# antofuller/jumbo_mae_tpu

Hardware: AMD Instinct MI355X
Metric: pretrain images/sec (whole node) ViT-L/16 224 mask75% at 1/2/4/8 MI355X (higher is better)
Workload: dtype bf16; 1 GPU; model=vit_large_patch16 jumbo-MAE (3 CLS, shared jumbo MLP) + decoder 8x512x16h, global_batch=4096, seq_len=52, decoder_seq_len=199, parallelism=dp1, per_gpu_batch=4096, grad_accum=2, micro_batch=2048, grad_ckpt=False, hip_graph=False, optimizer=adamw(0.9,0.95) wd0.05 warmup-cosine

## Files before the change

jumbo_mae_tpu_amd/csrc/bindings.cpp:

```cpp
#include <torch/extension.h>
#include <c10/hip/HIPStream.h>
#include <hip/hip_runtime.h>

#include <climits>

#include "jm_api.h"

namespace {

hipStream_t stream() { return c10::hip::getCurrentHIPStream().stream(); }

#define CHECK_CUDA(x) TORCH_CHECK((x).is_cuda(), #x " must be a GPU tensor")
#define CHECK_CONTIG(x) TORCH_CHECK((x).is_contiguous(), #x " must be contiguous")
#define CHECK_DT(x, d) TORCH_CHECK((x).scalar_type() == (d), #x " has wrong dtype")

const uint16_t* bf(const torch::Tensor& t) { return reinterpret_cast<const uint16_t*>(t.data_ptr()); }
uint16_t* bfm(torch::Tensor& t) { return reinterpret_cast<uint16_t*>(t.data_ptr()); }
uint16_t* bfp(const torch::Tensor& t) { return reinterpret_cast<uint16_t*>(t.data_ptr()); }
const float* fopt(const c10::optional<torch::Tensor>& t) {
  return t.has_value() && t->defined() ? t->data_ptr<float>() : nullptr;
}
float* fopt_m(c10::optional<torch::Tensor>& t) { return t.has_value() && t->defined() ? t->data_ptr<float>() : nullptr; }

void check_rc(int rc, const char* what) { TORCH_CHECK(rc == 0, what, ": unsupported shape (rc=", rc, ")"); }
// ... 1546 lines not shown
  m.def("attn_max_seq", &jm_attn_max_seq);
  m.def("attn_head_dims", &attn_head_dims);
  m.def("attn_fused_bias", &attn_fused_bias, py::arg("S"), py::arg("hd"));
  m.def("attn_dropout", &attn_dropout, py::arg("S"), py::arg("hd"));
  m.def("gemm_tn_wgrad", &gemm_tn_wgrad, py::arg("dy"), py::arg("x"), py::arg("g"), py::arg("store") = false);
  m.def("gemm_tn_wgrad_seg", &gemm_tn_wgrad_seg, py::arg("dys"), py::arg("xs"), py::arg("g"), py::arg("store") = false);
  m.def("zero_ranges", &zero_ranges, "zero float ranges of a flat buffer (one launch)");
  m.def("colsum_add_f32", &colsum_add_f32, "g += x.sum(0) for a row-strided fp32 [rows, n] view");
  m.def("gemm_tn_wgrad_seg_group", &gemm_tn_wgrad_seg_group, py::arg("dys"), py::arg("xs"), py::arg("gs"),
        py::arg("stores") = std::vector<bool>{}, "grouped segmented weight gradients (<= 2 problems)");
  m.def("gemm_tn_wgrad_group", &gemm_tn_wgrad_group, py::arg("dys"), py::arg("xs"), py::arg("gs"),
        py::arg("stores") = std::vector<bool>{}, "grouped weight gradients over one M (<= 4 problems)");
  m.def("gemm_test_force", &jm_gemm_test_force, py::arg("path"), py::arg("rows") = 0,
        "numerics tests only: NT GEMM kernel path 0 = by shape, 1 = 64-deep main loop everywhere, "
        "2 = 4-phase kernels at every M without tail split (rows = forced tile height)");
  m.def("gemm_nt_tiles", &jm_gemm_nt_tiles, py::arg("M"), py::arg("N"), py::arg("K") = 1024, py::arg("epi") = 0,
        py::arg("lda") = 0, "output tiles (workgroups before split-K) of an NT launch");
  m.def(
      "gemm_nt_tail_plan",
      [](int M, int N, int K, int epi, long lda) {
        int r = 0;
        long n = 0;
        const int S = jm_gemm_nt_tail_plan(M, N, K, epi, lda, &r, &n);
        return std::make_pair(S, r);
      },
      py::arg("M"), py::arg("N"), py::arg("K"), py::arg("epi") = 0, py::arg("lda") = 0,
      "(S, tail tiles) of the tail split of an NT launch (S = 0: none); read-only");
  m.def("transpose_bf16_batch", &transpose_bf16_batch);
  m.def("gemm_nt_splitk", &gemm_nt_splitk, py::arg("A"), py::arg("B"), py::arg("bias") = py::none(),
        py::arg("splits") = 8, py::arg("add") = py::none());
// ... 62 lines not shown
```

jumbo_mae_tpu_amd/csrc/common.h:

```cpp
#pragma once
#include <hip/hip_runtime.h>
#include <hip/hip_bf16.h>
#include <stdint.h>

#include "jm_api.h"

#define JM_DEVICE __device__ __forceinline__

typedef __attribute__((ext_vector_type(8))) __bf16 bf16x8_t;
typedef __attribute__((ext_vector_type(4))) float f32x4_t;
typedef __attribute__((ext_vector_type(4))) short s16x4_t;
typedef __attribute__((ext_vector_type(8))) short s16x8_t;
typedef uint16_t bf16_raw;

constexpr int WAVE = 64;

JM_DEVICE float bf2f(uint16_t v) { return __uint_as_float(((uint32_t)v) << 16); }

JM_DEVICE uint32_t drop_hash(uint32_t j, uint64_t seed) {
  uint32_t x = (j + (uint32_t)seed) ^ (uint32_t)(seed >> 32);
  x ^= x >> 16;
  x *= 0x7feb352du;
  x ^= x >> 15;
  x *= 0x846ca68bu;
// ... 95 lines not shown
template <int B>
JM_DEVICE uint32_t gd_put(float d, uint32_t w) { return __builtin_amdgcn_cvt_pk_u8_f32(__builtin_fmaf(d, GD_Q, (float)GD_Z), B, w); }
JM_DEVICE uint2 gd_pack8(const float* d) {
  uint2 v;
  v.x = gd_put<3>(d[3], gd_put<2>(d[2], gd_put<1>(d[1], gd_put<0>(d[0], 0u))));
  v.y = gd_put<3>(d[7], gd_put<2>(d[6], gd_put<1>(d[5], gd_put<0>(d[4], 0u))));
  return v;
}
JM_DEVICE void gd_unpack4(uint32_t w, float s, float* d) {
  d[0] = ((float)(w & 255u) - (float)GD_Z) * s;
  d[1] = ((float)((w >> 8) & 255u) - (float)GD_Z) * s;
  d[2] = ((float)((w >> 16) & 255u) - (float)GD_Z) * s;
  d[3] = ((float)(w >> 24) - (float)GD_Z) * s;
}

template <int CTRL>
JM_DEVICE float dpp_mov(float v) {
  return __builtin_bit_cast(float, __builtin_amdgcn_update_dpp(0, __builtin_bit_cast(int, v), CTRL, 0xF, 0xF, true));
}

template <int CTRL>
JM_DEVICE uint32_t dpp_mov_u32(uint32_t v) {
  return (uint32_t)__builtin_amdgcn_update_dpp(0, (int)v, CTRL, 0xF, 0xF, true);
}

JM_DEVICE float row16_sum(float v) {
  v += dpp_mov<0xB1>(v);
  v += dpp_mov<0x4E>(v);
  v += dpp_mov<0x141>(v);
  v += dpp_mov<0x140>(v);
// ... 111 lines not shown
```

jumbo_mae_tpu_amd/csrc/gemm.hip:

```cpp
#include <type_traits>

#include "common.h"
#include "jm_api.h"

namespace {

constexpr int BM = 256, BN = 256;
constexpr size_t GEMM_SMEM = 128 * 1024;

typedef __attribute__((address_space(3))) void lds_void_t;

JM_DEVICE __amdgpu_buffer_rsrc_t make_rsrc(const uint16_t* base, long bytes) {
  const int n = bytes >= 0xffffffffL ? -1 : (int)bytes;
  return __builtin_amdgcn_make_buffer_rsrc((void*)base, (short)0, n, 0x00020000);
}

JM_DEVICE void blds16(__amdgpu_buffer_rsrc_t r, uint32_t voff, uint32_t soff, uint16_t* l) {
  __builtin_amdgcn_raw_ptr_buffer_load_lds(r, (lds_void_t*)(l), 16, voff, soff, 0, 0);
}

JM_DEVICE bf16x8_t lds8(const uint16_t* p) { return *reinterpret_cast<const bf16x8_t*>(p); }

JM_DEVICE f32x4_t mfma16(bf16x8_t a, bf16x8_t b, f32x4_t c) {
  return __builtin_amdgcn_mfma_f32_16x16x32_bf16(a, b, c, 0, 0, 0);
// ... 12 lines not shown

namespace {

template <int W>
JM_DEVICE void gelu_d_drop(const GemmEpi& ep, long idx0, float* g, float* d) {
  const uint64_t seed = (uint64_t)ep.dseed[0];
#pragma unroll
  for (int j = 0; j < W; j += 2) {
    const uint32_t h = drop_hash((uint32_t)((idx0 + j) >> 1), seed);
    const bool k0 = drop_keep_half(h, 0, ep.dthr), k1 = drop_keep_half(h, 1, ep.dthr);
    g[j] = k0 ? g[j] * ep.dscale : 0.f;
    d[j] = k0 ? d[j] : 0.f;
    g[j + 1] = k1 ? g[j + 1] * ep.dscale : 0.f;
    d[j + 1] = k1 ? d[j + 1] : 0.f;
  }
}

template <int EPI, int NTW, int MTW = 8>
JM_DEVICE void epilogue(const f32x4_t (&acc)[8][NTW], const GemmEpi& ep, int M, int N, int mb, int nb, int l16,
                        int g) {
#pragma unroll
  for (int nt = 0; nt < NTW; ++nt) {
    const int n = nb + nt * 16 + 4 * g;
    if (n >= N) continue;
    float bv[4] = {0.f, 0.f, 0.f, 0.f};
    if (ep.bias) load4(ep.bias + n, bv);
#pragma unroll
    for (int mt = 0; mt < MTW; ++mt) {
      const int m = mb + mt * 16 + l16;
      if (m >= M) continue;
// ... 64 lines not shown
}

template <typename T>
JM_DEVICE void st16(T* p, uint4 v, bool nts) {
  typedef __attribute__((ext_vector_type(4))) unsigned int u32x4_t;
  if (nts) __builtin_nontemporal_store(u32x4_t{v.x, v.y, v.z, v.w}, reinterpret_cast<u32x4_t*>(p));
  else *reinterpret_cast<uint4*>(p) = v;
}

JM_DEVICE void st8(uint8_t* p, uint2 v, bool nts) {
  typedef __attribute__((ext_vector_type(2))) unsigned int u32x2_t;
  if (nts) __builtin_nontemporal_store(u32x2_t{v.x, v.y}, reinterpret_cast<u32x2_t*>(p));
  else *reinterpret_cast<uint2*>(p) = v;
}

JM_DEVICE uint4 pack8(const float* f) {
  uint4 v;
  v.x = pack_bf2(f[0], f[1]);
  v.y = pack_bf2(f[2], f[3]);
  v.z = pack_bf2(f[4], f[5]);
  v.w = pack_bf2(f[6], f[7]);
  return v;
}

template <int EPI, int NTW, int NTH, int BNT = BN, bool NTS = false, int TR = BM>
JM_DEVICE void epilogue_lds(const f32x4_t (&acc)[8][NTW], const GemmEpi& ep, uint16_t* cs, int M, int N, int m0,
                            int n0, int wr, int wc, int l16, int g) {
  constexpr int RB = BNT;
  constexpr int HR = TR / 2, MTW = HR / 16;
  asm volatile("s_waitcnt vmcnt(0) lgkmcnt(0)\n\ts_barrier" ::: "memory");
  constexpr int LPR = BNT / 8;
  constexpr int RPP = NTH / LPR;
  int tid = threadIdx.x;
  asm volatile("" : "+v"(tid));
  const int c = tid % LPR;
  const bool col_ok = n0 + c * 8 < N;
  constexpr bool PRE = EPI == EPI_DGELU || EPI == EPI_DMUL;
  constexpr int NPASS = PRE ? TR / RPP : 1;
  constexpr int PF = NPASS < 8 ? NPASS : 8;
  uint4 auxv[PF];
  auto aux_load = [&](int i) {
    const int m = m0 + tid / LPR + i * RPP;
// ... 48 lines not shown
        }
        uint4 o;
        uint32_t* ow = reinterpret_cast<uint32_t*>(&o);
#pragma unroll
        for (int j = 0; j < 8; j += 2) {
          const float a0 = bf2f(dg[j]) * (EPI == EPI_DMUL ? hp[j] : gd[j]);
          const float a1 = bf2f(dg[j + 1]) * (EPI == EPI_DMUL ? hp[j + 1] : gd[j + 1]);
          ow[j / 2] = pack_bf2(a0, a1);
          f[j] = __uint_as_float(ow[j / 2] << 16);
          f[j + 1] = __uint_as_float(ow[j / 2] & 0xffff0000u);
          csum[j] += f[j];
          csum[j + 1] += f[j + 1];
        }
        st16(ep.out + (long)m * ep.ldo + n0 + c * 8, o, NTS);
      } else if (EPI == EPI_GELU_D) {
        float fh[8], fg[8], fd[8];
        const uint16_t* h = reinterpret_cast<const uint16_t*>(&v);
#pragma unroll
        for (int j = 0; j < 8; ++j) fh[j] = bf2f(h[j]);
        gelu_n<8, true, true>(fh, fg, fd);
        if (ep.dseed) gelu_d_drop<8>(ep, (long)m * ep.ldo + n0 + c * 8, fg, fd);
        st8(ep.dq + (long)m * ep.ldo + n0 + c * 8, gd_pack8(fd), NTS);
        st16(ep.out2 + (long)m * ep.ldo + n0 + c * 8, pack8(fg), NTS);
      } else if (EPI == EPI_GELU_ONLY) {
        float fh[8], f[8];
        const uint16_t* h = reinterpret_cast<const uint16_t*>(&v);
#pragma unroll
        for (int j = 0; j < 8; ++j) fh[j] = bf2f(h[j]);
        gelu_n<8, true, false>(fh, f, nullptr);
        st16(ep.out + (long)m * ep.ldo + n0 + c * 8, pack8(f), NTS);
      } else {
        st16(ep.out + (long)m * ep.ldo + n0 + c * 8, v, NTS);
      }
      if (EPI == EPI_GELU) {
        float fh[8], f[8];
        const uint16_t* h = reinterpret_cast<const uint16_t*>(&v);
#pragma unroll
        for (int j = 0; j < 8; ++j) fh[j] = bf2f(h[j]);
        gelu_n<8, true, false>(fh, f, nullptr);
        st16(ep.out2 + (long)m * ep.ldo + n0 + c * 8, pack8(f), NTS);
      }
    }
  };
  if constexpr (PRE) {
#pragma unroll
    for (int i = 0; i < NPASS; ++i) {
      pass(tid / LPR + i * RPP, auxv[i % PF]);
      if (i + PF < NPASS) auxv[i % PF] = aux_load(i + PF);
    }
  } else {
#pragma unroll 4
    for (int r = tid / LPR; r < TR; r += RPP) pass(r, auxv[0]);
  }
  if ((EPI == EPI_DGELU || EPI == EPI_DMUL) && ep.colpart != nullptr) {
    float* red = reinterpret_cast<float*>(cs);
    __syncthreads();
// ... 107 lines not shown
      __builtin_amdgcn_sched_barrier(0);
      if constexpr (KIND == 2) issue(u + 2);
      read(u + 1, H0{}, f0);
      mfma_rows(R4{}, f1);
      interleave();
    } else {
      mfma_rows(R4{}, f1);
    }
    __builtin_amdgcn_sched_barrier(0);
  };
  using K2 = std::integral_constant<int, 2>;
  using K1 = std::integral_constant<int, 1>;
  using K0 = std::integral_constant<int, 0>;

  const int nst = K / BK2;
  issue(0);
  if (nst > 1) {
    issue(1);
    asm volatile("s_waitcnt vmcnt(8)\n\ts_barrier" ::: "memory");
  } else {
    asm volatile("s_waitcnt vmcnt(0)\n\ts_barrier" ::: "memory");
  }
  __builtin_amdgcn_sched_barrier(0);
  Frags<NTW> f0, f1;
  read(0, H0{}, f0);
  int u = 0;
  for (; u + 2 < nst; ++u) stage(K2{}, u, f0, f1);
  if (u + 1 < nst) stage(K1{}, u++, f0, f1);
  stage(K0{}, u, f0, f1);

// ... 12 lines not shown
  } else if (EPI == EPI_PARTIAL) {
    float* dst = ep.part + (long)split * M * N;
#pragma unroll
    for (int mt = 0; mt < 8; ++mt) {
      const int m = m0 + wr * 128 + mt * 16 + l16;
      if (m >= M) continue;
#pragma unroll
      for (int nt = 0; nt < NTW; ++nt) {
        const int n = n0 + wc * NTW * 16 + nt * 16 + 4 * g;
        if (n >= N) continue;
        float v[4] = {acc[mt][nt][0], acc[mt][nt][1], acc[mt][nt][2], acc[mt][nt][3]};
        store4(dst + (long)m * N + n, v);
      }
    }
  } else if (N % 8 == 0)
    epilogue_lds<EPI, NTW, 512, BN, NTS>(acc, ep, smem, M, N, m0, n0, wr, wc, l16, g);
  else
    epilogue<EPI, NTW>(acc, ep, M, N, m0 + wr * 128, n0 + wc * NTW * 16, l16, g);
}

template <int EPI, bool NTS>
__global__ __launch_bounds__(512, 1) void gemm_nt64_kernel(const uint16_t* __restrict__ A, long lda,
                                                           const uint16_t* __restrict__ B, long ldb, int M, int N,
                                                           int K, GemmEpi ep, int GROUP_M) {
  JM_DGUARD(blockDim.x == 512 && K % 64 == 0 && M > 0 && N > 0);
  extern __shared__ __attribute__((aligned(16))) uint16_t smem[];
  nt64_body<EPI, NTS>(A, lda, B, ldb, M, N, K, ep, GROUP_M, smem);
}

template <int MTL>
__attribute__((always_inline)) JM_DEVICE void p4_mainloop(const uint16_t* __restrict__ A, long lda,
// ... 147 lines not shown
  sync(I3{});
  issue(1, I2{});
  read_a(0, I0{}, ax);
  read_b(0, I0{}, bp);
  int t = 0;
  for (; t + 4 <= nk; t += 2) {
    tile(K2{}, t, bp, bq);
    tile(K2{}, t + 1, bq, bp);
  }
  tile(K1{}, t, bp, bq);
  tile(K0{}, t + 1, bq, bp);
}

template <int EPI, int MTL>
__attribute__((always_inline)) JM_DEVICE void p4_epilogue(const f32x4_t (&acc)[8][4], const GemmEpi& ep, int M,
                                                          int N, int m0, int n0, int split, uint16_t* smem) {
  constexpr int NTW = 4, WN = 4;
  constexpr int HR = 64 + 16 * MTL, MTW = 4 + MTL;
  const int tid = threadIdx.x;
  const int wave = __builtin_amdgcn_readfirstlane(tid >> 6), lane = tid & 63;
  const int l16 = lane & 15, g = lane >> 4;
  const int wr = wave / WN, wc = wave % WN;
  if (EPI == EPI_PARTIAL) {
    float* dst = ep.part + (long)split * M * N;
#pragma unroll
    for (int mt = 0; mt < MTW; ++mt) {
      const int m = m0 + wr * HR + mt * 16 + l16;
      if (m >= M) continue;
#pragma unroll
      for (int nt = 0; nt < NTW; ++nt) {
        const int n = n0 + wc * NTW * 16 + nt * 16 + 4 * g;
        if (n >= N) continue;
        float v[4] = {acc[mt][nt][0], acc[mt][nt][1], acc[mt][nt][2], acc[mt][nt][3]};
        store4(dst + (long)m * N + n, v);
      }
    }
  } else if (N % 8 == 0)
    epilogue_lds<EPI, NTW, 512, BN, true, 2 * HR>(acc, ep, smem, M, N, m0, n0, wr, wc, l16, g);
  else
    epilogue<EPI, NTW, MTW>(acc, ep, M, N, m0 + wr * HR, n0 + wc * NTW * 16, l16, g);
}

template <int EPI, int MTL = 4>
__global__ __launch_bounds__(512, 1) void gemm_p4_kernel(const uint16_t* __restrict__ A, long lda,
                                                         const uint16_t* __restrict__ B, long ldb, int M, int N,
                                                         int K, GemmEpi ep, int GROUP_M) {
  JM_DGUARD(blockDim.x == 512 && K % 128 == 0 && M > 0 && N > 0);
  extern __shared__ __attribute__((aligned(16))) uint16_t smem[];
  if (__builtin_amdgcn_readfirstlane(threadIdx.x) >= 256) __builtin_amdgcn_s_setprio(1);
  int m0, n0, split = 0;
  if (EPI != EPI_PARTIAL && ep.t_count > 0) {
    int tg;
    tile_of_range(M, N, GROUP_M, ep.t_begin, ep.t_count, 1, m0, n0, split, tg);
  } else {
    tile_of<BN, 128 + 32 * MTL>(M, N, GROUP_M, m0, n0, EPI == EPI_PARTIAL ? ep.splits : 1,
                                EPI == EPI_PARTIAL ? &split : nullptr);
  }
  int k_begin = 0;
  if (EPI == EPI_PARTIAL) {
    const int ku = K / 128;
    const int ku0 = split * ku / ep.splits, ku1 = (split + 1) * ku / ep.splits;
    k_begin = ku0 * 128;
    K = (ku1 - ku0) * 128;
  }
  f32x4_t acc[8][4];
  p4_mainloop<MTL>(A, lda, B, ldb, M, N, m0, n0, k_begin, K, acc, smem);
  p4_epilogue<EPI, MTL>(acc, ep, M, N, m0, n0, split, smem);
}

constexpr int NBM = 128, NBN = 192, NKT = 64;
constexpr int N_AEL = NBM * NKT, N_BEL = NBN * NKT, N_STAGE = N_AEL + N_BEL;
constexpr int N_RING = 3;
constexpr int N_LD = NBN + 8;
static_assert(N_RING * N_STAGE * 2 <= (int)GEMM_SMEM, "narrow ring exceeds the LDS budget");

JM_DEVICE void narrow_tile(int M, int N, int GROUP_M, int splits, int& m0, int& n0, int& split) {
  const int nM = (M + NBM - 1) / NBM, nN = (N + NBN - 1) / NBN;
  const int tiles = nM * nN, nwg = tiles * splits;
  const int orig = blockIdx.x;
  const int xcd = orig & 7, q = nwg >> 3, r = nwg & 7;
  int wg = (xcd < r ? xcd * (q + 1) : r * (q + 1) + (xcd - r) * q) + (orig >> 3);
  split = wg / tiles;
  wg -= split * tiles;
  const int per_group = GROUP_M * nN;
  const int first_m = (wg / per_group) * GROUP_M;
  const int gsz = min(nM - first_m, GROUP_M);
  m0 = (first_m + (wg % per_group) % gsz) * NBM;
  n0 = ((wg % per_group) / gsz) * NBN;
}

template <int EPI>
JM_DEVICE void narrow_epilogue(const f32x4_t (&acc)[4][3], const GemmEpi& ep, uint16_t* cs, int M, int N, int m0,
                               int n0, int split, int wr, int wc, int l16, int g) {
  if constexpr (EPI == EPI_PARTIAL) {
    float* dst = ep.part + (long)split * M * N;
#pragma unroll
    for (int mt = 0; mt < 4; ++mt) {
      const int m = m0 + wr * 64 + mt * 16 + l16;
      if (m >= M) continue;
#pragma unroll
      for (int nt = 0; nt < 3; ++nt) {
        const int n = n0 + wc * 48 + nt * 16 + 4 * g;
        if (n >= N) continue;
        float v[4] = {acc[mt][nt][0], acc[mt][nt][1], acc[mt][nt][2], acc[mt][nt][3]};
        store4(dst + (long)m * N + n, v);
      }
    }
    return;
// ... 52 lines not shown
          gd_unpack4(auxv[i].x, ep.dqs, hp);
          gd_unpack4(auxv[i].y, ep.dqs, hp + 4);
        } else {
          const uint16_t* ah = reinterpret_cast<const uint16_t*>(&auxv[i]);
#pragma unroll
          for (int j = 0; j < 8; ++j) hp[j] = bf2f(ah[j]);
          gelu_n<8, false, true>(hp, nullptr, gd);
        }
#pragma unroll
        for (int j = 0; j < 8; ++j) {
          f[j] = bf2f(f2bf(bf2f(h[j]) * (EPI == EPI_DMUL ? hp[j] : gd[j])));
          csum[j] += f[j];
        }
        st16(o, pack8(f), false);
      } else if constexpr (EPI == EPI_GELU_D) {
        float fh[8], fg[8], fd[8];
#pragma unroll
        for (int j = 0; j < 8; ++j) fh[j] = bf2f(h[j]);
        gelu_n<8, true, true>(fh, fg, fd);
        if (ep.dseed) gelu_d_drop<8>(ep, (long)m * ep.ldo + n, fg, fd);
        st8(ep.dq + (long)m * ep.ldo + n, gd_pack8(fd), false);
        st16(ep.out2 + (long)m * ep.ldo + n, pack8(fg), false);
      } else if constexpr (EPI == EPI_GELU_ONLY) {
        float fh[8], f[8];
#pragma unroll
        for (int j = 0; j < 8; ++j) fh[j] = bf2f(h[j]);
        gelu_n<8, true, false>(fh, f, nullptr);
        st16(o, pack8(f), false);
      } else {
        st16(o, v, false);
        if constexpr (EPI == EPI_GELU) {
          float fh[8], f[8];
#pragma unroll
          for (int j = 0; j < 8; ++j) fh[j] = bf2f(h[j]);
          gelu_n<8, true, false>(fh, f, nullptr);
          st16(ep.out2 + (long)m * ep.ldo + n, pack8(f), false);
        }
      }
    }
  }
  if constexpr (PRE) {
    if (ep.colpart != nullptr) {
      float* red = reinterpret_cast<float*>(cs);
      __syncthreads();
      if (active) {
#pragma unroll
        for (int j = 0; j < 8; ++j) red[rr * NBN + c * 8 + j] = csum[j];
      }
      __syncthreads();
      if (tid < NBN && n0 + tid < N) {
        float a = 0.f;
#pragma unroll
// ... 43 lines not shown
    uint16_t* lb = la + N_AEL;
#pragma unroll
    for (int p = 0; p < 2; ++p) blds16(ra, a_src[p], k0b, la + (wave + 8 * p) * 8 * NKT);
#pragma unroll
    for (int p = 0; p < 3; ++p) blds16(rb, b_src[p], k0b, lb + (wave + 8 * p) * 8 * NKT);
  };
  const int ch0 = ((0 * 4 + g) ^ swz64(l16)) * 8, ch1 = ((1 * 4 + g) ^ swz64(l16)) * 8;
  const int a_row = (wr * 64 + l16) * NKT, b_row = N_AEL + (wc * 48 + l16) * NKT;
  f32x4_t acc[4][3];
#pragma unroll
  for (int i = 0; i < 4; ++i)
#pragma unroll
    for (int j = 0; j < 3; ++j) acc[i][j] = f32x4_t{0.f, 0.f, 0.f, 0.f};

  const int nk = K / NKT;
  issue(0);
  if (nk > 1) issue(1);
  for (int t = 0; t < nk; ++t) {
    if (t + 1 < nk) asm volatile("s_waitcnt vmcnt(5) lgkmcnt(0)\n\ts_barrier" ::: "memory");
    else asm volatile("s_waitcnt vmcnt(0) lgkmcnt(0)\n\ts_barrier" ::: "memory");
    __builtin_amdgcn_sched_barrier(0);
    if (t + 2 < nk) issue(t + 2);
    const uint16_t* base = smem + (t % N_RING) * N_STAGE;
    bf16x8_t a[4][2], b[3][2];
#pragma unroll
    for (int kk = 0; kk < 2; ++kk) {
      const int ch = kk ? ch1 : ch0;
#pragma unroll
      for (int nt = 0; nt < 3; ++nt) b[nt][kk] = lds8(base + b_row + nt * 16 * NKT + ch);
#pragma unroll
// ... 3 lines not shown
    for (int kk = 0; kk < 2; ++kk)
#pragma unroll
      for (int mt = 0; mt < 4; ++mt)
#pragma unroll
        for (int nt = 0; nt < 3; ++nt) acc[mt][nt] = mfma16(b[nt][kk], a[mt][kk], acc[mt][nt]);
    __builtin_amdgcn_sched_group_barrier(0x100, 7, 0);
#pragma unroll
    for (int i = 0; i < 7; ++i) {
      __builtin_amdgcn_sched_group_barrier(0x008, 1, 0);
      __builtin_amdgcn_sched_group_barrier(0x100, 1, 0);
    }
    __builtin_amdgcn_sched_group_barrier(0x008, 17, 0);
    __builtin_amdgcn_sched_barrier(0);
  }
  if (wave >= 4) __builtin_amdgcn_s_setprio(0);
  narrow_epilogue<EPI>(acc, ep, smem, M, N, m0, n0, split, wr, wc, l16, g);
}

template <int EPI>
__global__ __launch_bounds__(256) void tail_finish_kernel(GemmEpi ep, int M, int N, int GROUP_M) {
  __shared__ float red[8][BN];
  const int tg = blockIdx.x >> 3, rb = blockIdx.x & 7;
  int m0, n0;
  tile_coords(ep.t_begin + tg, M, N, GROUP_M, m0, n0);
  const int tid = threadIdx.x, c = tid & 31, rr = tid >> 5;
  const int n = n0 + c * 8;
  float csum[8] = {0.f, 0.f, 0.f, 0.f, 0.f, 0.f, 0.f, 0.f};
  float bv[8] = {0.f, 0.f, 0.f, 0.f, 0.f, 0.f, 0.f, 0.f};
  if (ep.bias && n < N) load8(ep.bias + n, bv);
#pragma unroll
  for (int i = 0; i < 4; ++i) {
// ... 61 lines not shown
    int dev = 0;
    (void)hipGetDevice(&dev);
    hipDeviceProp_t prop;
    (void)hipGetDeviceProperties(&prop, dev);
    g_num_cus = prop.multiProcessorCount;
  }
  return g_num_cus;
}

template <int EPI, bool NTS>
void launch_nt64(const uint16_t* A, long lda, const uint16_t* B, long ldb, int M, int N, int K, const GemmEpi& ep,
                 int nwg, hipStream_t st) {
  static bool attr = false;
  if (!attr) {
    (void)hipFuncSetAttribute((const void*)gemm_nt64_kernel<EPI, NTS>, hipFuncAttributeMaxDynamicSharedMemorySize,
                              (int)GEMM_SMEM);
    attr = true;
  }
  gemm_nt64_kernel<EPI, NTS><<<nwg, 512, GEMM_SMEM, st>>>(A, lda, B, ldb, M, N, K, ep, GEMM_GROUP);
}

template <int EPI, int MTL>
void launch_p4(const uint16_t* A, long lda, const uint16_t* B, long ldb, int M, int N, int K, const GemmEpi& ep,
               int nwg, hipStream_t st) {
  static bool attr = false;
  if (!attr) {
    (void)hipFuncSetAttribute((const void*)gemm_p4_kernel<EPI, MTL>, hipFuncAttributeMaxDynamicSharedMemorySize,
                              (int)GEMM_SMEM);
    attr = true;
  }
  gemm_p4_kernel<EPI, MTL><<<nwg, 512, GEMM_SMEM, st>>>(A, lda, B, ldb, M, N, K, ep, GEMM_GROUP);
}

template <int EPI>
void launch_narrow(const uint16_t* A, long lda, const uint16_t* B, long ldb, int M, int N, int K, const GemmEpi& ep,
                   hipStream_t st) {
  static bool attr = false;
  constexpr size_t sm = (size_t)N_RING * N_STAGE * 2;
  if (!attr) {
    (void)hipFuncSetAttribute((const void*)gemm_narrow_kernel<EPI>, hipFuncAttributeMaxDynamicSharedMemorySize,
                              (int)sm);
    attr = true;
  }
  const int nwg = ((M + NBM - 1) / NBM) * ((N + NBN - 1) / NBN) * (EPI == EPI_PARTIAL ? ep.splits : 1);
  gemm_narrow_kernel<EPI><<<nwg, 512, sm, st>>>(A, lda, B, ldb, M, N, K, ep, GEMM_GROUP);
}

constexpr int NARROW_MAX_M = 4096;

bool p4_ok(int K, int epi, int splits) {
  return g_test_path != 1 && K % 128 == 0 && (epi != EPI_PARTIAL || K / 128 >= splits);
}

// ... 55 lines not shown

template <int EPI>
void launch_tail(const uint16_t* A, long lda, const uint16_t* B, long ldb, int M, int N, int K, const GemmEpi& ep,
                 int tiles, hipStream_t st) {
  const int r = ep.t_count;
  GemmEpi em = ep;
  em.t_begin = 0;
  em.t_count = tiles - r;
  launch_epi<EPI>(A, lda, B, ldb, M, N, K, em, tiles - r, st);
  GemmEpi et = ep;
  et.t_begin = tiles - r;
  launch_nt64<EPI_TAIL, false>(A, lda, B, ldb, M, N, K, et, r * ep.tail_S, st);
  tail_finish_kernel<EPI><<<r * 8, 256, 0, st>>>(et, M, N, GEMM_GROUP);
}

}

void jm_gemm_test_force(int path, int rows) {
  g_test_path = (path == 1 || path == 2) ? path : 0;
  g_test_rows = (g_test_path == 2 && (rows == 224 || rows == 192 || rows == 160 || rows == 256)) ? rows : 0;
}

int jm_gemm_nt_tiles(int M, int N, int K, int epi, long lda) {
  if (narrow(M, N, K, epi)) return ((M + NBM - 1) / NBM) * ((N + NBN - 1) / NBN);
  const int tr = tile_rows(M, N, K, epi, lda);
  return ((M + tr - 1) / tr) * ((N + BN - 1) / BN);
}

int jm_gemm_nt_colpart_rows(int M, int N, int K, int epi, long lda) {
  if (narrow(M, N, K, epi)) return (M + NBM - 1) / NBM;
// ... 19 lines not shown
  *tail_r = r;
  return S;
}
}

int jm_gemm_nt_tail_plan(int M, int N, int K, int epi, long lda, int* tail_r, long* ws_floats) {
  *tail_r = 0;
  *ws_floats = 0;
  if (tile_rows(M, N, K, epi, lda) != BM) return 0;
  const int S = tail_plan_256(M, N, K, epi, tail_r);
  *ws_floats = (long)S * *tail_r * BM * BN;
  return S;
}

int jm_gemm_nt(const uint16_t* A, long lda, const uint16_t* B, long ldb, int M, int N, int K, int epi,
               const GemmEpi& ep, hipStream_t st) {
  if (K % 64 || N % 4 || M <= 0 || N <= 0) return -1;
  if ((long)M * lda * 2 >= (1L << 32) || (long)N * ldb * 2 >= (1L << 32)) return -2;
  const int nwg = ((M + BM - 1) / BM) * ((N + BN - 1) / BN) * (epi == EPI_PARTIAL ? ep.splits : 1);
  if (epi == EPI_PARTIAL && (ep.splits < 1 || (K / 64) < ep.splits)) return -4;
  if (ep.tail != nullptr && ep.tail_S >= 2 && ep.t_count > 0) {
    const int tiles = ((M + BM - 1) / BM) * ((N + BN - 1) / BN);
    if (epi == EPI_STORE) launch_tail<EPI_STORE>(A, lda, B, ldb, M, N, K, ep, tiles, st);
    else if (epi == EPI_GELU) launch_tail<EPI_GELU>(A, lda, B, ldb, M, N, K, ep, tiles, st);
    else if (epi == EPI_DGELU) launch_tail<EPI_DGELU>(A, lda, B, ldb, M, N, K, ep, tiles, st);
    else if (epi == EPI_GELU_ONLY) launch_tail<EPI_GELU_ONLY>(A, lda, B, ldb, M, N, K, ep, tiles, st);
    else return -3;
    return 0;
  }
  if (epi == EPI_PARTIAL)
    launch_epi<EPI_PARTIAL>(A, lda, B, ldb, M, N, K, ep, nwg, st);
  else if (epi == EPI_STORE)
// ... 18 lines not shown
```

jumbo_mae_tpu_amd/csrc/jm_api.h:

```cpp
#pragma once
#include <cstddef>
#include <cstdint>

#include <hip/hip_runtime.h>

struct JmDrop {
  const int64_t* seed;
  uint32_t thr;
  float scale;
  long ioff;
};

struct JmLnRes {
  const uint16_t* y;
  uint16_t* dy;
  long yB, yT;
  const float* scale;
  const float* mask;
  int T0;
  float* dscale;
  float* dbias;
  JmDrop drop;
};

// ... 21 lines not shown
  uint16_t* out2;
  const uint16_t* aux;
  float* colpart;
  float* part;
  int splits;
  float* tail;
  int tail_S;
  int t_begin;
  int t_count;
  const int64_t* dseed;
  uint32_t dthr;
  float dscale;
  uint8_t* dq;
  const uint8_t* dqa;
  float dqs;
};


int jm_layernorm_fwd(const float* x, long sB, long sT, int B, int T, int D, const float* gamma, const float* beta,
                     float eps, void* y, int out_bf16, float* mean, float* rstd, hipStream_t st, uint16_t* y2 = nullptr);
int jm_layernorm_bwd(const void* dy, int dy_bf16, const float* x, long sB, long sT, int B, int T, int D,
                     const float* mean, const float* rstd, const float* gamma, float* dx_ptr, long oB, long oT,
                     const float* dres, long rB, long rT, float* dgamma, float* dbeta, int accum_params, float* ws,
                     const JmLnRes* res, hipStream_t st, const uint16_t* hx = nullptr,
                     const float* beta = nullptr);
int jm_layernorm_bwd_blocks(int rows, int D);
int jm_residual_ln_fwd(const float* x, long sB, long sT, const uint16_t* y, const float* scale, const float* mask,
                       float* x1, long oB, long oT, uint16_t* h, float* mean, float* rstd, int B, int T, int T0,
                       int D, const float* gamma, const float* beta, float eps, hipStream_t st, int R0 = 0,
                       JmDrop drop = JmDrop{nullptr, 0u, 1.f, 0});
// ... 77 lines not shown
int jm_patch_mse_bwd(const uint16_t* pred, long ldp, const uint8_t* img, const float* dmse, uint16_t* dpred, long rows,
                     int N, int H, int W, int p, int norm_pix, hipStream_t st);
int jm_debug_line_mae();

int jm_recon(const void* pred, int pred_bf16, const uint8_t* img, const float* mask, long maskB, uint8_t* recon,
             uint8_t* paste, uint8_t* masked, float* err, int B, int H, int W, int p, int norm_pix, int fill,
             hipStream_t st);
int jm_debug_line_recon();

int jm_gemm_nt(const uint16_t* A, long lda, const uint16_t* B, long ldb, int M, int N, int K, int epi,
               const GemmEpi& ep, hipStream_t st);
int jm_gemm_nt_tiles(int M, int N, int K, int epi, long lda);
int jm_gemm_nt_colpart_rows(int M, int N, int K, int epi, long lda);
int jm_gemm_nt_tail_plan(int M, int N, int K, int epi, long lda, int* tail_r, long* ws_floats);
void jm_gemm_test_force(int path, int rows);
int jm_debug_line_gemm();

size_t jm_gemm_tn_smem();
int jm_gemm_tn_plan(const TnGroup& grp, int M, int* S_out);
int jm_gemm_tn(const TnGroup& grp, const TnSegs* segs, int M, int sps, int S, hipStream_t st, int store);
int jm_debug_line_gemm_tn();

int jm_dropout_apply(const void* x, void* y, long n, int bf16, const int64_t* seed, uint32_t thr, float scale,
                     hipStream_t st);
int jm_gelu_drop(const uint16_t* h, uint16_t* g, uint16_t* gp, long n, const int64_t* seed, uint32_t thr, float scale,
                 hipStream_t st);
int jm_softmax_dropout_fwd(const float* z, float* p, float* pd, long rows, int S, const int64_t* seed, uint32_t thr,
                           float scale, hipStream_t st);
int jm_softmax_dropout_bwd(const float* dpd, const float* p, float* dz, long rows, int S, const int64_t* seed,
                           uint32_t thr, float scale, hipStream_t st);
// ... 51 lines not shown
```

Measured before the change: 6718 images/sec.

## Evaluate GELU epilogues through an LDS-resident bf16 lookup table

Builds a one-time per-device table mapping bf16 inputs within an exponent window to the packed bf16 GELU value and the 8-bit derivative code. The GEMM kernels stage it into LDS above the tile ring and replace the per-element erf/tanh arithmetic in the GELU epilogues with table lookups, falling back to arithmetic when any input in a group of eight lies outside the window. This removes VALU transcendental work from the epilogue. In exchange each workgroup spends 32 KB more LDS and a staging load, which may lower occupancy, and adds LDS traffic. It is disabled when dropout seeds are present.

After: 6744 images/sec (median of 6 runs). Within noise of the previous version (+0.4%).

```diff
diff --git a/jumbo_mae_tpu_amd/csrc/bindings.cpp b/jumbo_mae_tpu_amd/csrc/bindings.cpp
--- a/jumbo_mae_tpu_amd/csrc/bindings.cpp
+++ b/jumbo_mae_tpu_amd/csrc/bindings.cpp
@@ -1584,6 +1584,22 @@
   m.def("gemm_test_force", &jm_gemm_test_force, py::arg("path"), py::arg("rows") = 0,
         "numerics tests only: NT GEMM kernel path 0 = by shape, 1 = 64-deep main loop everywhere, "
         "2 = 4-phase kernels at every M without tail split (rows = forced tile height)");
+  m.def("gelu_table_enable", &jm_gelu_table_enable, py::arg("on") = -1,
+        "GELU epilogues through the lookup table (1) or arithmetic (0); returns the previous setting, on < 0 reads it");
+  m.def(
+      "gelu_eval",
+      [](torch::Tensor h, bool table) {
+        CHECK_DT(h, torch::kBFloat16);
+        TORCH_CHECK(h.is_cuda() && h.is_contiguous() && h.numel() > 0 && h.numel() % 8 == 0,
+                    "gelu_eval: contiguous device bf16, numel % 8 == 0");
+        auto g = torch::empty_like(h);
+        auto q = torch::empty(h.sizes(), h.options().dtype(torch::kUInt8));
+        check_rc(jm_gelu_eval(bf(h), bfm(g), q.data_ptr<uint8_t>(), h.numel(), table ? 1 : 0, stream()), "gelu_eval");
+        return std::make_pair(g, q);
+      },
+      py::arg("h"), py::arg("table"),
+      "numerics tests only: (bf16 gelu(h), gelu'(h) codes) elementwise through the GELU epilogues' table path "
+      "(lookup + out-of-window arithmetic) or their arithmetic alone");
   m.def("gemm_nt_tiles", &jm_gemm_nt_tiles, py::arg("M"), py::arg("N"), py::arg("K") = 1024, py::arg("epi") = 0,
         py::arg("lda") = 0, "output tiles (workgroups before split-K) of an NT launch");
   m.def(
diff --git a/jumbo_mae_tpu_amd/csrc/common.h b/jumbo_mae_tpu_amd/csrc/common.h
--- a/jumbo_mae_tpu_amd/csrc/common.h
+++ b/jumbo_mae_tpu_amd/csrc/common.h
@@ -133,6 +133,41 @@
   d[3] = ((float)(w >> 24) - (float)GD_Z) * s;
 }
 
+constexpr int GT_ELO = 99, GT_EXPS = 32;
+constexpr int GT_IDX_BITS = 14;
+static_assert(GT_EXPS * 128 * 4 == 1 << GT_IDX_BITS, "GT_IDX_BITS");
+constexpr int GT_ENTRIES = 2 * GT_EXPS * 128;
+constexpr int GT_BYTES = GT_ENTRIES * 4;
+constexpr uint32_t GT_LO4 = (uint32_t)GT_ELO << 9;
+constexpr uint32_t GT_OUT_MASK = (1u << 17) - (1u << GT_IDX_BITS);
+JM_DEVICE uint32_t gt_offset(uint32_t x) {
+  return (x & ((1u << GT_IDX_BITS) - 4u)) | ((x >> (17 - GT_IDX_BITS)) & (1u << GT_IDX_BITS));
+}
+JM_DEVICE uint32_t gt_lookup2(const uint32_t* tab, uint32_t w, uint32_t& t0, uint32_t& t1) {
+  const uint32_t x0 = (w << 2) - GT_LO4, x1 = (w >> 14) - GT_LO4;
+  t0 = *reinterpret_cast<const uint32_t*>(reinterpret_cast<const char*>(tab) + gt_offset(x0));
+  t1 = *reinterpret_cast<const uint32_t*>(reinterpret_cast<const char*>(tab) + gt_offset(x1));
+  return x0 | x1;
+}
+JM_DEVICE uint32_t gt_gelu2(uint32_t t0, uint32_t t1) { return __builtin_amdgcn_perm(t1, t0, 0x07060302u); }
+JM_DEVICE uint32_t gt_code4(uint32_t t0, uint32_t t1, uint32_t t2, uint32_t t3) {
+  return __builtin_amdgcn_perm(__builtin_amdgcn_perm(t3, t2, 0x04000c0cu), __builtin_amdgcn_perm(t1, t0, 0x0c0c0400u),
+                               0x07060100u);
+}
+JM_DEVICE bool gt_lookup8(const uint32_t* tab, const uint4& v, uint32_t* t) {
+  uint32_t any = gt_lookup2(tab, v.x, t[0], t[1]);
+  any |= gt_lookup2(tab, v.y, t[2], t[3]);
+  any |= gt_lookup2(tab, v.z, t[4], t[5]);
+  any |= gt_lookup2(tab, v.w, t[6], t[7]);
+  return (any & GT_OUT_MASK) == 0;
+}
+JM_DEVICE uint4 gt_gelu8(const uint32_t* t) {
+  return make_uint4(gt_gelu2(t[0], t[1]), gt_gelu2(t[2], t[3]), gt_gelu2(t[4], t[5]), gt_gelu2(t[6], t[7]));
+}
+JM_DEVICE uint2 gt_code8(const uint32_t* t) {
+  return make_uint2(gt_code4(t[0], t[1], t[2], t[3]), gt_code4(t[4], t[5], t[6], t[7]));
+}
+
 template <int CTRL>
 JM_DEVICE float dpp_mov(float v) {
   return __builtin_bit_cast(float, __builtin_amdgcn_update_dpp(0, __builtin_bit_cast(int, v), CTRL, 0xF, 0xF, true));
diff --git a/jumbo_mae_tpu_amd/csrc/gemm.hip b/jumbo_mae_tpu_amd/csrc/gemm.hip
--- a/jumbo_mae_tpu_amd/csrc/gemm.hip
+++ b/jumbo_mae_tpu_amd/csrc/gemm.hip
@@ -7,6 +7,7 @@
 
 constexpr int BM = 256, BN = 256;
 constexpr size_t GEMM_SMEM = 128 * 1024;
+static_assert(GEMM_SMEM + GT_BYTES <= 160 * 1024, "ring + GELU table exceed the CU's LDS");
 
 typedef __attribute__((address_space(3))) void lds_void_t;
 
@@ -50,6 +51,61 @@
     g[j + 1] = k1 ? g[j + 1] * ep.dscale : 0.f;
     d[j + 1] = k1 ? d[j + 1] : 0.f;
   }
+}
+
+template <int EPI>
+constexpr bool epi_table = EPI == EPI_GELU || EPI == EPI_GELU_ONLY || EPI == EPI_GELU_D;
+template <int EPI>
+constexpr size_t epi_table_bytes = epi_table<EPI> ? (size_t)GT_BYTES : 0;
+
+JM_DEVICE void gt_stage(const uint32_t* gtab, uint16_t* ltab) {
+  static_assert(GT_BYTES % (512 * 16) == 0, "whole rounds");
+  const int tid = threadIdx.x;
+  const int wave = __builtin_amdgcn_readfirstlane(tid >> 6), lane = tid & 63;
+  const __amdgpu_buffer_rsrc_t r = make_rsrc(reinterpret_cast<const uint16_t*>(gtab), GT_BYTES);
+#pragma unroll
+  for (int i = 0; i < GT_BYTES / (512 * 16); ++i)
+    blds16(r, (uint32_t)((i * 512 + wave * 64 + lane) * 16), 0, ltab + (i * 512 + wave * 64) * 8);
+}
+
+JM_DEVICE uint4 pack8(const float* f) {
+  uint4 v;
+  v.x = pack_bf2(f[0], f[1]);
+  v.y = pack_bf2(f[2], f[3]);
+  v.z = pack_bf2(f[4], f[5]);
+  v.w = pack_bf2(f[6], f[7]);
+  return v;
+}
+
+JM_DEVICE void gelu_d8(const uint4& v, uint4& o, uint2& q) {
+  float fh[8], fg[8], fd[8];
+  const uint16_t* h = reinterpret_cast<const uint16_t*>(&v);
+#pragma unroll
+  for (int j = 0; j < 8; ++j) fh[j] = bf2f(h[j]);
+  gelu_n<8, true, true>(fh, fg, fd);
+  q = gd_pack8(fd);
+  o = pack8(fg);
+}
+JM_DEVICE uint4 gelu8(const uint4& v) {
+  float fh[8], f[8];
+  const uint16_t* h = reinterpret_cast<const uint16_t*>(&v);
+#pragma unroll
+  for (int j = 0; j < 8; ++j) fh[j] = bf2f(h[j]);
+  gelu_n<8, true, false>(fh, f, nullptr);
+  return pack8(f);
+}
+JM_DEVICE void gelu_d8_tab(const uint32_t* tab, const uint4& v, uint4& o, uint2& q) {
+  uint32_t t[8];
+  if (gt_lookup8(tab, v, t)) {
+    o = gt_gelu8(t);
+    q = gt_code8(t);
+  } else {
+    gelu_d8(v, o, q);
+  }
+}
+JM_DEVICE uint4 gelu8_tab(const uint32_t* tab, const uint4& v) {
+  uint32_t t[8];
+  return gt_lookup8(tab, v, t) ? gt_gelu8(t) : gelu8(v);
 }
 
 template <int EPI, int NTW, int MTW = 8>
@@ -144,18 +200,9 @@
   else *reinterpret_cast<uint2*>(p) = v;
 }
 
-JM_DEVICE uint4 pack8(const float* f) {
-  uint4 v;
-  v.x = pack_bf2(f[0], f[1]);
-  v.y = pack_bf2(f[2], f[3]);
-  v.z = pack_bf2(f[4], f[5]);
-  v.w = pack_bf2(f[6], f[7]);
-  return v;
-}
-
 template <int EPI, int NTW, int NTH, int BNT = BN, bool NTS = false, int TR = BM>
 JM_DEVICE void epilogue_lds(const f32x4_t (&acc)[8][NTW], const GemmEpi& ep, uint16_t* cs, int M, int N, int m0,
-                            int n0, int wr, int wc, int l16, int g) {
+                            int n0, int wr, int wc, int l16, int g, const uint32_t* tab = nullptr) {
   constexpr int RB = BNT;
   constexpr int HR = TR / 2, MTW = HR / 16;
   asm volatile("s_waitcnt vmcnt(0) lgkmcnt(0)\n\ts_barrier" ::: "memory");
@@ -234,32 +281,30 @@
         }
         st16(ep.out + (long)m * ep.ldo + n0 + c * 8, o, NTS);
       } else if (EPI == EPI_GELU_D) {
-        float fh[8], fg[8], fd[8];
-        const uint16_t* h = reinterpret_cast<const uint16_t*>(&v);
-#pragma unroll
-        for (int j = 0; j < 8; ++j) fh[j] = bf2f(h[j]);
-        gelu_n<8, true, true>(fh, fg, fd);
-        if (ep.dseed) gelu_d_drop<8>(ep, (long)m * ep.ldo + n0 + c * 8, fg, fd);
-        st8(ep.dq + (long)m * ep.ldo + n0 + c * 8, gd_pack8(fd), NTS);
-        st16(ep.out2 + (long)m * ep.ldo + n0 + c * 8, pack8(fg), NTS);
+        uint4 o;
+        uint2 q;
+        if (tab) {
+          gelu_d8_tab(tab, v, o, q);
+        } else if (ep.dseed) {
+          float fh[8], fg[8], fd[8];
+          const uint16_t* h = reinterpret_cast<const uint16_t*>(&v);
+#pragma unroll
+          for (int j = 0; j < 8; ++j) fh[j] = bf2f(h[j]);
+          gelu_n<8, true, true>(fh, fg, fd);
+          gelu_d_drop<8>(ep, (long)m * ep.ldo + n0 + c * 8, fg, fd);
+          q = gd_pack8(fd);
+          o = pack8(fg);
+        } else {
+          gelu_d8(v, o, q);
+        }
+        st8(ep.dq + (long)m * ep.ldo + n0 + c * 8, q, NTS);
+        st16(ep.out2 + (long)m * ep.ldo + n0 + c * 8, o, NTS);
       } else if (EPI == EPI_GELU_ONLY) {
-        float fh[8], f[8];
-        const uint16_t* h = reinterpret_cast<const uint16_t*>(&v);
-#pragma unroll
-        for (int j = 0; j < 8; ++j) fh[j] = bf2f(h[j]);
-        gelu_n<8, true, false>(fh, f, nullptr);
-        st16(ep.out + (long)m * ep.ldo + n0 + c * 8, pack8(f), NTS);
+        st16(ep.out + (long)m * ep.ldo + n0 + c * 8, tab ? gelu8_tab(tab, v) : gelu8(v), NTS);
       } else {
         st16(ep.out + (long)m * ep.ldo + n0 + c * 8, v, NTS);
       }
-      if (EPI == EPI_GELU) {
-        float fh[8], f[8];
-        const uint16_t* h = reinterpret_cast<const uint16_t*>(&v);
-#pragma unroll
-        for (int j = 0; j < 8; ++j) fh[j] = bf2f(h[j]);
-        gelu_n<8, true, false>(fh, f, nullptr);
-        st16(ep.out2 + (long)m * ep.ldo + n0 + c * 8, pack8(f), NTS);
-      }
+      if (EPI == EPI_GELU) st16(ep.out2 + (long)m * ep.ldo + n0 + c * 8, tab ? gelu8_tab(tab, v) : gelu8(v), NTS);
     }
   };
   if constexpr (PRE) {
@@ -397,6 +442,13 @@
   using K0 = std::integral_constant<int, 0>;
 
   const int nst = K / BK2;
+  const uint32_t* tab = nullptr;
+  if constexpr (epi_table<EPI>) {
+    if (ep.gtab) {
+      gt_stage(ep.gtab, smem + GEMM_SMEM / 2);
+      tab = reinterpret_cast<const uint32_t*>(smem + GEMM_SMEM / 2);
+    }
+  }
   issue(0);
   if (nst > 1) {
     issue(1);
@@ -439,7 +491,7 @@
       }
     }
   } else if (N % 8 == 0)
-    epilogue_lds<EPI, NTW, 512, BN, NTS>(acc, ep, smem, M, N, m0, n0, wr, wc, l16, g);
+    epilogue_lds<EPI, NTW, 512, BN, NTS>(acc, ep, smem, M, N, m0, n0, wr, wc, l16, g, tab);
   else
     epilogue<EPI, NTW>(acc, ep, M, N, m0 + wr * 128, n0 + wc * NTW * 16, l16, g);
 }
@@ -617,7 +669,8 @@
 
 template <int EPI, int MTL>
 __attribute__((always_inline)) JM_DEVICE void p4_epilogue(const f32x4_t (&acc)[8][4], const GemmEpi& ep, int M,
-                                                          int N, int m0, int n0, int split, uint16_t* smem) {
+                                                          int N, int m0, int n0, int split, uint16_t* smem,
+                                                          const uint32_t* tab) {
   constexpr int NTW = 4, WN = 4;
   constexpr int HR = 64 + 16 * MTL, MTW = 4 + MTL;
   const int tid = threadIdx.x;
@@ -639,7 +692,7 @@
       }
     }
   } else if (N % 8 == 0)
-    epilogue_lds<EPI, NTW, 512, BN, true, 2 * HR>(acc, ep, smem, M, N, m0, n0, wr, wc, l16, g);
+    epilogue_lds<EPI, NTW, 512, BN, true, 2 * HR>(acc, ep, smem, M, N, m0, n0, wr, wc, l16, g, tab);
   else
     epilogue<EPI, NTW, MTW>(acc, ep, M, N, m0 + wr * HR, n0 + wc * NTW * 16, l16, g);
 }
@@ -666,9 +719,16 @@
     k_begin = ku0 * 128;
     K = (ku1 - ku0) * 128;
   }
+  const uint32_t* tab = nullptr;
+  if constexpr (epi_table<EPI>) {
+    if (ep.gtab) {
+      gt_stage(ep.gtab, smem + GEMM_SMEM / 2);
+      tab = reinterpret_cast<const uint32_t*>(smem + GEMM_SMEM / 2);
+    }
+  }
   f32x4_t acc[8][4];
   p4_mainloop<MTL>(A, lda, B, ldb, M, N, m0, n0, k_begin, K, acc, smem);
-  p4_epilogue<EPI, MTL>(acc, ep, M, N, m0, n0, split, smem);
+  p4_epilogue<EPI, MTL>(acc, ep, M, N, m0, n0, split, smem, tab);
 }
 
 constexpr int NBM = 128, NBN = 192, NKT = 64;
@@ -676,6 +736,7 @@
 constexpr int N_RING = 3;
 constexpr int N_LD = NBN + 8;
 static_assert(N_RING * N_STAGE * 2 <= (int)GEMM_SMEM, "narrow ring exceeds the LDS budget");
+static_assert((N_RING * N_STAGE * 2) % 16 == 0, "the GELU table above the ring is 16-byte aligned");
 
 JM_DEVICE void narrow_tile(int M, int N, int GROUP_M, int splits, int& m0, int& n0, int& split) {
   const int nM = (M + NBM - 1) / NBM, nN = (N + NBN - 1) / NBN;
@@ -694,7 +755,7 @@
 
 template <int EPI>
 JM_DEVICE void narrow_epilogue(const f32x4_t (&acc)[4][3], const GemmEpi& ep, uint16_t* cs, int M, int N, int m0,
-                               int n0, int split, int wr, int wc, int l16, int g) {
+                               int n0, int split, int wr, int wc, int l16, int g, const uint32_t* tab) {
   if constexpr (EPI == EPI_PARTIAL) {
     float* dst = ep.part + (long)split * M * N;
 #pragma unroll
@@ -777,28 +838,28 @@
         }
         st16(o, pack8(f), false);
       } else if constexpr (EPI == EPI_GELU_D) {
-        float fh[8], fg[8], fd[8];
-#pragma unroll
-        for (int j = 0; j < 8; ++j) fh[j] = bf2f(h[j]);
-        gelu_n<8, true, true>(fh, fg, fd);
-        if (ep.dseed) gelu_d_drop<8>(ep, (long)m * ep.ldo + n, fg, fd);
-        st8(ep.dq + (long)m * ep.ldo + n, gd_pack8(fd), false);
-        st16(ep.out2 + (long)m * ep.ldo + n, pack8(fg), false);
+        uint4 og;
+        uint2 q;
+        if (tab) {
+          gelu_d8_tab(tab, v, og, q);
+        } else if (ep.dseed) {
+          float fh[8], fg[8], fd[8];
+#pragma unroll
+          for (int j = 0; j < 8; ++j) fh[j] = bf2f(h[j]);
+          gelu_n<8, true, true>(fh, fg, fd);
+          gelu_d_drop<8>(ep, (long)m * ep.ldo + n, fg, fd);
+          q = gd_pack8(fd);
+          og = pack8(fg);
+        } else {
+          gelu_d8(v, og, q);
+        }
+        st8(ep.dq + (long)m * ep.ldo + n, q, false);
+        st16(ep.out2 + (long)m * ep.ldo + n, og, false);
       } else if constexpr (EPI == EPI_GELU_ONLY) {
-        float fh[8], f[8];
-#pragma unroll
-        for (int j = 0; j < 8; ++j) fh[j] = bf2f(h[j]);
-        gelu_n<8, true, false>(fh, f, nullptr);
-        st16(o, pack8(f), false);
+        st16(o, tab ? gelu8_tab(tab, v) : gelu8(v), false);
       } else {
         st16(o, v, false);
-        if constexpr (EPI == EPI_GELU) {
-          float fh[8], f[8];
-#pragma unroll
-          for (int j = 0; j < 8; ++j) fh[j] = bf2f(h[j]);
-          gelu_n<8, true, false>(fh, f, nullptr);
-          st16(ep.out2 + (long)m * ep.ldo + n, pack8(f), false);
-        }
+        if constexpr (EPI == EPI_GELU) st16(ep.out2 + (long)m * ep.ldo + n, tab ? gelu8_tab(tab, v) : gelu8(v), false);
       }
     }
   }
@@ -872,6 +933,13 @@
     for (int j = 0; j < 3; ++j) acc[i][j] = f32x4_t{0.f, 0.f, 0.f, 0.f};
 
   const int nk = K / NKT;
+  const uint32_t* tab = nullptr;
+  if constexpr (epi_table<EPI>) {
+    if (ep.gtab) {
+      gt_stage(ep.gtab, smem + N_RING * N_STAGE);
+      tab = reinterpret_cast<const uint32_t*>(smem + N_RING * N_STAGE);
+    }
+  }
   issue(0);
   if (nk > 1) issue(1);
   for (int t = 0; t < nk; ++t) {
@@ -905,7 +973,7 @@
     __builtin_amdgcn_sched_barrier(0);
   }
   if (wave >= 4) __builtin_amdgcn_s_setprio(0);
-  narrow_epilogue<EPI>(acc, ep, smem, M, N, m0, n0, split, wr, wc, l16, g);
+  narrow_epilogue<EPI>(acc, ep, smem, M, N, m0, n0, split, wr, wc, l16, g, tab);
 }
 
 template <int EPI>
@@ -997,10 +1065,11 @@
   static bool attr = false;
   if (!attr) {
     (void)hipFuncSetAttribute((const void*)gemm_nt64_kernel<EPI, NTS>, hipFuncAttributeMaxDynamicSharedMemorySize,
-                              (int)GEMM_SMEM);
+                              (int)(GEMM_SMEM + epi_table_bytes<EPI>));
     attr = true;
   }
-  gemm_nt64_kernel<EPI, NTS><<<nwg, 512, GEMM_SMEM, st>>>(A, lda, B, ldb, M, N, K, ep, GEMM_GROUP);
+  gemm_nt64_kernel<EPI, NTS><<<nwg, 512, GEMM_SMEM + epi_table_bytes<EPI>, st>>>(A, lda, B, ldb, M, N, K, ep,
+                                                                                   GEMM_GROUP);
 }
 
 template <int EPI, int MTL>
@@ -1009,17 +1078,18 @@
   static bool attr = false;
   if (!attr) {
     (void)hipFuncSetAttribute((const void*)gemm_p4_kernel<EPI, MTL>, hipFuncAttributeMaxDynamicSharedMemorySize,
-                              (int)GEMM_SMEM);
+                              (int)(GEMM_SMEM + epi_table_bytes<EPI>));
     attr = true;
   }
-  gemm_p4_kernel<EPI, MTL><<<nwg, 512, GEMM_SMEM, st>>>(A, lda, B, ldb, M, N, K, ep, GEMM_GROUP);
+  gemm_p4_kernel<EPI, MTL><<<nwg, 512, GEMM_SMEM + epi_table_bytes<EPI>, st>>>(A, lda, B, ldb, M, N, K, ep,
+                                                                                 GEMM_GROUP);
 }
 
 template <int EPI>
 void launch_narrow(const uint16_t* A, long lda, const uint16_t* B, long ldb, int M, int N, int K, const GemmEpi& ep,
                    hipStream_t st) {
   static bool attr = false;
-  constexpr size_t sm = (size_t)N_RING * N_STAGE * 2;
+  constexpr size_t sm = (size_t)N_RING * N_STAGE * 2 + epi_table_bytes<EPI>;
   if (!attr) {
     (void)hipFuncSetAttribute((const void*)gemm_narrow_kernel<EPI>, hipFuncAttributeMaxDynamicSharedMemorySize,
                               (int)sm);
@@ -1105,6 +1175,76 @@
   tail_finish_kernel<EPI><<<r * 8, 256, 0, st>>>(et, M, N, GEMM_GROUP);
 }
 
+__global__ __launch_bounds__(256) void gelu_table_kernel(uint32_t* tab) {
+  const int i = blockIdx.x * 256 + threadIdx.x;
+  if (i >= GT_ENTRIES / 8) return;
+  const uint32_t e0 = 8u * i;
+  const uint32_t b0 = ((e0 >> (GT_IDX_BITS - 2)) << 15) | ((e0 & ((1u << (GT_IDX_BITS - 2)) - 1u)) + (GT_ELO << 7));
+  uint32_t w[4];
+#pragma unroll
+  for (int j = 0; j < 4; ++j) w[j] = (b0 + 2 * j) | ((b0 + 2 * j + 1) << 16);
+  uint4 o;
+  uint2 q;
+  gelu_d8(make_uint4(w[0], w[1], w[2], w[3]), o, q);
+  const uint16_t* gh = reinterpret_cast<const uint16_t*>(&o);
+  const uint8_t* qc = reinterpret_cast<const uint8_t*>(&q);
+#pragma unroll
+  for (int j = 0; j < 8; ++j) tab[e0 + j] = ((uint32_t)gh[j] << 16) | qc[j];
+}
+
+__global__ __launch_bounds__(256) void gelu_eval_kernel(const uint16_t* h, uint16_t* g, uint8_t* q, long n8,
+                                                        const uint32_t* tab) {
+  const long i = (long)blockIdx.x * 256 + threadIdx.x;
+  if (i >= n8) return;
+  const uint4 v = *reinterpret_cast<const uint4*>(h + 8 * i);
+  uint4 o;
+  uint2 c;
+  if (tab) gelu_d8_tab(tab, v, o, c);
+  else gelu_d8(v, o, c);
+  *reinterpret_cast<uint4*>(g + 8 * i) = o;
+  *reinterpret_cast<uint2*>(q + 8 * i) = c;
+}
+
+constexpr int GT_MAX_DEV = 64;
+uint32_t* g_gtab[GT_MAX_DEV] = {};
+int g_gtab_on = -1;
+
+const uint32_t* gelu_table(hipStream_t st) {
+  int dev = 0;
+  if (hipGetDevice(&dev) != hipSuccess || dev < 0 || dev >= GT_MAX_DEV) return nullptr;
+  if (g_gtab[dev]) return g_gtab[dev];
+  hipStreamCaptureStatus cs = hipStreamCaptureStatusNone;
+  if (hipStreamIsCapturing(st, &cs) != hipSuccess || cs != hipStreamCaptureStatusNone) return nullptr;
+  uint32_t* t = nullptr;
+  if (hipMalloc(&t, GT_BYTES) != hipSuccess) return nullptr;
+  gelu_table_kernel<<<(GT_ENTRIES / 8 + 255) / 256, 256, 0, st>>>(t);
+  if (hipStreamSynchronize(st) != hipSuccess) {
+    (void)hipFree(t);
+    return nullptr;
+  }
+  g_gtab[dev] = t;
+  return t;
+}
+
+}
+
+int jm_gelu_table_enable(int on) {
+  if (g_gtab_on < 0) {
+    const char* e = getenv("JMAE_GELU_TABLE");
+    g_gtab_on = (e && e[0] == '0') ? 0 : 1;
+  }
+  const int was = g_gtab_on;
+  if (on >= 0) g_gtab_on = on ? 1 : 0;
+  return was;
+}
+
+int jm_gelu_eval(const uint16_t* h, uint16_t* g, uint8_t* q, long n, int table, hipStream_t st) {
+  if (n <= 0 || n % 8) return -1;
+  const uint32_t* tab = nullptr;
+  if (table && (tab = gelu_table(st)) == nullptr) return -2;
+  const long n8 = n / 8;
+  gelu_eval_kernel<<<(int)((n8 + 255) / 256), 256, 0, st>>>(h, g, q, n8, tab);
+  return 0;
 }
 
 void jm_gemm_test_force(int path, int rows) {
@@ -1154,8 +1294,13 @@
 }
 
 int jm_gemm_nt(const uint16_t* A, long lda, const uint16_t* B, long ldb, int M, int N, int K, int epi,
-               const GemmEpi& ep, hipStream_t st) {
+               const GemmEpi& ep_in, hipStream_t st) {
   if (K % 64 || N % 4 || M <= 0 || N <= 0) return -1;
+  GemmEpi ep = ep_in;
+  ep.gtab = nullptr;
+  if ((epi == EPI_GELU || epi == EPI_GELU_ONLY || epi == EPI_GELU_D) && !ep.dseed && N % 8 == 0 &&
+      jm_gelu_table_enable(-1))
+    ep.gtab = gelu_table(st);
   if ((long)M * lda * 2 >= (1L << 32) || (long)N * ldb * 2 >= (1L << 32)) return -2;
   const int nwg = ((M + BM - 1) / BM) * ((N + BN - 1) / BN) * (epi == EPI_PARTIAL ? ep.splits : 1);
   if (epi == EPI_PARTIAL && (ep.splits < 1 || (K / 64) < ep.splits)) return -4;
diff --git a/jumbo_mae_tpu_amd/csrc/jm_api.h b/jumbo_mae_tpu_amd/csrc/jm_api.h
--- a/jumbo_mae_tpu_amd/csrc/jm_api.h
+++ b/jumbo_mae_tpu_amd/csrc/jm_api.h
@@ -59,6 +59,7 @@
   uint8_t* dq;
   const uint8_t* dqa;
   float dqs;
+  const uint32_t* gtab;
 };
 
 
@@ -166,6 +167,8 @@
 int jm_gemm_nt_colpart_rows(int M, int N, int K, int epi, long lda);
 int jm_gemm_nt_tail_plan(int M, int N, int K, int epi, long lda, int* tail_r, long* ws_floats);
 void jm_gemm_test_force(int path, int rows);
+int jm_gelu_table_enable(int on);
+int jm_gelu_eval(const uint16_t* h, uint16_t* g, uint8_t* q, long n, int table, hipStream_t st);
 int jm_debug_line_gemm();
 
 size_t jm_gemm_tn_smem();
```
